# sparisi/pvr_habitat

Measured on AMD Instinct MI355X. Metric: frames/sec embedded (ResNet50, 256x256), higher is better.
Workload: dtype f16

## Files before the change

### include/pvr_hip.h

```cpp
#ifndef PVR_HIP_H
#define PVR_HIP_H

#include <stddef.h>
#include <stdint.h>

#ifdef __cplusplus
extern "C" {
#endif

typedef int pvr_status;
#define PVR_OK 0
#define PVR_ERR_INVALID 1
#define PVR_ERR_MISSING_WEIGHT 2
#define PVR_ERR_HIP 3
#define PVR_ERR_STATE 4

#define PVR_BF16 0
#define PVR_F16 1
#define PVR_F32 2

#define PVR_ARCH_RESNET50 0
#define PVR_ARCH_RESNET50_L4 1
#define PVR_ARCH_RESNET50_L3 2
#define PVR_ARCH_CLIP_VIT_B32 3
// ... 79 lines not shown
                             int32_t h, int32_t w, int32_t cin, int32_t cout, int32_t kh, int32_t kw, int32_t stride, int32_t pad, int32_t relu,
                             int32_t out_f32, int32_t dtype, void *hip_stream);
pvr_status pvr_op_conv2d_dual(const void *in_dev, const void *in2_dev, const void *wgt_dev, const float *bias_dev, void *out_dev, int32_t n, int32_t h,
                              int32_t w, int32_t cin, int32_t cout, int32_t kh, int32_t kw, int32_t stride, int32_t pad, int32_t h2, int32_t w2,
                              int32_t cin2, int32_t stride2, int32_t relu, int32_t dtype, void *hip_stream);
pvr_status pvr_op_conv_wfrag_pool(const void *in_dev, const void *wgt_packed_dev, const float *bias_dev, const void *residual_dev, float *pool_out_dev,
                                  int64_t pool_stride, int32_t n, int32_t cin, int32_t cout, int32_t dtype, void *hip_stream);
int64_t pvr_debug_conv_wfrag_launches(void);
pvr_status pvr_op_split16_pack_weights(const float *w_dev, void *out_dev, int32_t rows, int32_t k, void *hip_stream);
pvr_status pvr_op_conv2d_split16(const float *in_dev, const void *wgt_split_dev, const float *bias_dev, const float *residual_dev, float *out_dev, int32_t n,
                                 int32_t h, int32_t w, int32_t cin, int32_t cout, int32_t k, int32_t stride, int32_t pad, int32_t relu, void *hip_stream);
pvr_status pvr_op_conv2d_f32(const float *in_dev, const float *wgt_dev, const float *bias_dev, const float *residual_dev, float *out_dev, int32_t n,
                             int32_t h, int32_t w, int32_t cin, int32_t cout, int32_t k, int32_t stride, int32_t pad, int32_t relu, void *hip_stream);
int64_t pvr_debug_conv_split16_launches(void);
int64_t pvr_debug_chain_wave128_launches(void);
pvr_status pvr_debug_set_stem_regpool(int32_t mode);
pvr_status pvr_debug_set_conv_algo(int32_t algo);
pvr_status pvr_file_sizes(const char *const *paths, int32_t n, int64_t *sizes, int32_t threads);
pvr_status pvr_read_files(const char *const *paths, int32_t n, uint8_t *dst, const int64_t *offsets, int32_t threads);
pvr_status pvr_stage_copy(void *dst, const void *src, int64_t rows, int64_t row_bytes, int64_t src_row_stride, int64_t run_bytes,
                          int64_t run_stride, int32_t threads);
int64_t pvr_png_scratch_bytes(int32_t n, int32_t h, int32_t w);
pvr_status pvr_png_decode(const uint8_t *files_dev, const int64_t *offsets_dev, int32_t n, int32_t h, int32_t w, uint8_t *out_dev,
                          uint8_t *scratch_dev, int64_t scratch_bytes, int32_t *status_dev, void *hip_stream);

int64_t pvr_debug_conv_expand_launches(void);
int64_t pvr_debug_pp_persistent_launches(void);
pvr_status pvr_op_avgpool(const void *in_dev, float *out_dev, int64_t out_stride, int32_t n, int32_t hw,
                          int32_t c, int32_t in_f32, int32_t dtype, void *hip_stream);
pvr_status pvr_op_nonfinite_flag(const float *x_dev, int64_t rows, int64_t cols, int64_t stride, int32_t *flag_dev, void *hip_stream);
// ... 9 lines not shown
```

### pvr_habitat_amd/_lib.py

```python
import ctypes as C
import os

_HERE = os.path.dirname(os.path.abspath(__file__))
LIB_PATH = os.environ.get('PVR_LIB') or os.path.join(_HERE, 'lib', 'libpvr_hip.so')

PVR_BF16, PVR_F16, PVR_F32 = 0, 1, 2
ARCH_RESNET50, ARCH_RESNET50_L4, ARCH_RESNET50_L3 = 0, 1, 2


class EncoderDesc(C.Structure):
    _fields_ = [('arch', C.c_int32), ('dtype', C.c_int32), ('max_batch', C.c_int32), ('chunk', C.c_int32),
                ('resize', C.c_int32), ('crop', C.c_int32), ('mean', C.c_float * 3), ('std_', C.c_float * 3)]


_lib = None

_SIGS = {
    'pvr_version': (C.c_char_p, []),
    'pvr_has_experiments': (C.c_int32, []),
    'pvr_debug_stem_u8_geometry_ok': (C.c_int32, [C.c_void_p, C.c_int32, C.c_int32, C.c_int32, C.c_int32]),
    'pvr_encoder_set_host_backend': (C.c_int, [C.c_void_p, C.c_int32]),
    'pvr_stage_copy': (C.c_int, [C.c_void_p, C.c_void_p, C.c_int64, C.c_int64, C.c_int64, C.c_int64, C.c_int64, C.c_int32]),
    'pvr_last_error': (C.c_size_t, [C.c_char_p, C.c_size_t]),
    'pvr_encoder_create': (C.c_int, [C.POINTER(EncoderDesc), C.POINTER(C.c_void_p)]),
# ... 34 lines not shown
    'pvr_op_conv_wfrag': (C.c_int, [C.c_void_p] * 5 + [C.c_int32] * 12 + [C.c_void_p]),
    'pvr_debug_conv_wfrag_launches': (C.c_int64, []),
    'pvr_op_conv_wfrag_pool': (C.c_int, [C.c_void_p] * 5 + [C.c_int64] + [C.c_int32] * 4 + [C.c_void_p]),
    'pvr_op_conv2d_dual': (C.c_int, [C.c_void_p] * 5 + [C.c_int32] * 15 + [C.c_void_p]),
    'pvr_op_pack_frag_weights': (C.c_int, [C.c_void_p, C.c_void_p, C.c_int32, C.c_int32, C.c_void_p]),
    'pvr_debug_bneck_frame_stamps': (C.c_int, [C.c_void_p] * 12 + [C.c_int32] * 2 + [C.c_void_p] * 2),
    'pvr_encoder_check_range': (C.c_int, [C.c_void_p, C.c_void_p, C.c_int32, C.c_int32, C.c_int32, C.c_void_p, C.c_int64, C.c_void_p, C.POINTER(C.c_int32)]),
    'pvr_encoder_debug_set_switch': (C.c_int, [C.c_void_p, C.c_char_p, C.c_int32]),
    'pvr_encoder_launch_kernel': (C.c_int32, [C.c_void_p, C.c_int32, C.c_int32, C.c_char_p, C.c_int32]),
    'pvr_op_split16_pack_weights': (C.c_int, [C.c_void_p, C.c_void_p, C.c_int32, C.c_int32, C.c_void_p]),
    'pvr_op_conv2d_split16': (C.c_int, [C.c_void_p] * 5 + [C.c_int32] * 9 + [C.c_void_p]),
    'pvr_op_conv2d_f32': (C.c_int, [C.c_void_p] * 5 + [C.c_int32] * 9 + [C.c_void_p]),
    'pvr_debug_conv_split16_launches': (C.c_int64, []),
    'pvr_debug_set_stem_regpool': (C.c_int, [C.c_int32]),
    'pvr_debug_chain_wave128_launches': (C.c_int64, []),
    'pvr_op_nonfinite_flag': (C.c_int, [C.c_void_p, C.c_int64, C.c_int64, C.c_int64, C.c_void_p, C.c_void_p]),
}


def lib():
    global _lib
    if _lib is None:
        if not os.path.isfile(LIB_PATH):
            raise RuntimeError('libpvr_hip.so not found at %s: build it with `make -C pvr_habitat_amd/csrc` '
                               '(there is no CPU fallback for the HIP path)' % LIB_PATH)
        l = C.CDLL(LIB_PATH)
        for name, (res, args) in _SIGS.items():
            if not hasattr(l, name):
                continue
            f = getattr(l, name)
# ... 26 lines not shown
```

### pvr_habitat_amd/csrc/api.hip

```cpp
#include <stdarg.h>
#include "common.h"
#include "sample_rng.h"
#include <dlfcn.h>

namespace pvr {

static thread_local std::string g_err;

void set_error(const char *fmt, ...) {
    char buf[1024];
    va_list ap;
    va_start(ap, fmt);
    vsnprintf(buf, sizeof buf, fmt, ap);
    va_end(ap);
    g_err = buf;
}
const std::string &last_error() { return g_err; }

namespace {
typedef int (*roctx_push_fn)(const char *);
typedef int (*roctx_pop_fn)();
struct Roctx {
    roctx_push_fn push = nullptr;
    roctx_pop_fn pop = nullptr;
// ... 34 lines not shown
                                int dtype, hipStream_t stream, unsigned long long *stamps);
void set_frame64(int mode);
long long bneck_frame64_launches();
long long pp_persistent_launches();
pvr_status launch_conv_pp256(const void *in, const void *wgt, const float *bias, const void *res, void *out, int n, int h, int w, int cin,
                             int cout, int kh, int kw, int stride, int pad, int act, int out_f32, int res_f32, int dtype, int bm, hipStream_t stream,
                             const void *in2 = nullptr, int h2 = 0, int w2 = 0, int cin2 = 0, int stride2 = 1);
long long conv_wfrag_launches();
pvr_status launch_conv_wfrag(const void *in, const void *wp, const float *bias, const void *res, void *out, int n, int h, int w, int cin, int cout,
                             int kh, int kw, int stride, int pad, int act, int out_f32, int dtype, hipStream_t stream, float *pool_out = nullptr,
                             int64_t pool_stride = 0);

void set_stem_regpool(int v);
long long conv_split16_launches();
long long chain_wave128_launches();
pvr_status launch_split16_pack(const float *w, void *out, int rows, int K, hipStream_t stream);
pvr_status launch_conv_split16(const float *in, const void *wsp, const float *bias, const float *res, float *out, int n, int h, int w, int cin,
                               int cout, int k, int stride, int pad, int relu, hipStream_t stream, float *out2 = nullptr, int n1 = 0, void *out16 = nullptr,
                               int terms = 3);
pvr_status launch_conv_f32(const float *, const float *, const float *, const float *, float *, int, int, int, int, int, int, int, int, int, hipStream_t);

static void *g_zero = nullptr;
static pvr_status zero_page(void **out) {
    if (!g_zero) {
        PVR_HIP_TRY(hipMalloc(&g_zero, 256));
        PVR_HIP_TRY(hipMemset(g_zero, 0, 256));
        PVR_HIP_TRY(hipDeviceSynchronize());
    }
    *out = g_zero;
    return PVR_OK;
// ... 65 lines not shown
    PVR_REQUIRE(n > 0 && h > 0 && w > 0, "pvr_op_conv2d_split16: empty input");
    return launch_conv_split16(in, wgt_split, bias, residual, out, n, h, w, cin, cout, k, stride, pad, relu, (hipStream_t)stream);
}
pvr_status pvr_op_conv2d_f32(const float *in, const float *wgt, const float *bias, const float *residual, float *out, int32_t n, int32_t h, int32_t w,
                             int32_t cin, int32_t cout, int32_t k, int32_t stride, int32_t pad, int32_t relu, void *stream) {
    PVR_REQUIRE(in && wgt && bias && out && n > 0, "pvr_op_conv2d_f32: null argument");
    return launch_conv_f32(in, wgt, bias, residual, out, n, h, w, cin, cout, k, stride, pad, relu, (hipStream_t)stream);
}
int64_t pvr_debug_conv_split16_launches(void) { return (int64_t)conv_split16_launches(); }
pvr_status pvr_debug_set_stem_regpool(int32_t mode) {
    PVR_REQUIRE(mode >= -1 && mode <= 1, "pvr_debug_set_stem_regpool: -1 (environment: PVR_STEM_REGPOOL, default on), 0 (LDS-tile pooling) or 1 (register pooling)");
    set_stem_regpool(mode);
    return PVR_OK;
}
int64_t pvr_debug_chain_wave128_launches(void) { return (int64_t)chain_wave128_launches(); }
int64_t pvr_debug_pp_persistent_launches(void) { return (int64_t)pp_persistent_launches(); }

size_t pvr_last_error(char *buf, size_t cap) {
    const std::string &e = last_error();
    if (buf && cap) {
        size_t n = e.size() < cap - 1 ? e.size() : cap - 1;
        memcpy(buf, e.data(), n);
        buf[n] = 0;
    }
    return e.size();
}

pvr_status pvr_op_preprocess(const uint8_t *frames, int32_t n, int32_t h, int32_t w, int32_t resize, int32_t crop,
                             void *out, int32_t dtype, void *stream) {
    PVR_REQUIRE(frames && out, "pvr_op_preprocess: null pointer");
// ... 83 lines not shown
```

### pvr_habitat_amd/csrc/bottleneck_chain.hip

```cpp
#include "chain_params.h"

namespace pvr {


__device__ __forceinline__ void ch_dma16(__amdgpu_buffer_rsrc_t rs, char *lds, int voff, int soff) {
    __builtin_amdgcn_raw_ptr_buffer_load_lds(rs, (__attribute__((address_space(3))) void *)lds, 16, voff, soff, 0, 0);
}

#ifdef CHAIN_STAMP
__device__ unsigned long long chain_stamps[8192][12];
#define CH_T(i_) { if (threadIdx.x == 0) ch_tt[i_] = __builtin_amdgcn_s_memrealtime(); }
#else
#define CH_T(i_)
#endif

#ifndef CH_KNOCK
#define CH_KNOCK 0
#endif
template <int AUX = 0>
__device__ __forceinline__ void store_b128_imm(u32x4 v, __amdgpu_buffer_rsrc_t rs, int voff, int imm) {
    if constexpr (!(CH_KNOCK & 1)) __builtin_amdgcn_raw_buffer_store_b128(v, rs, voff + imm, 0, AUX);
}

template <int CM, int CMN, bool F16, int RD, int OCC, bool HALO, bool DS = false, int PFK = -1>
// ... 561 lines not shown
    return !e || atoi(e) != 0;
}

bool chain_uses_wave_form(int cm, int cmn, int stride, bool ds) { return chain_wave_enabled() && chain_wave_supported(cm, cmn, stride, ds); }

bool chain_uses_wave128(int cm, int cmn, int stride, int64_t M) { return chain_wave_enabled() && chain_wave128_supported(cm, cmn, stride, M); }

bool chain_ds_supported(int cm, int cmn, int cin, int stride) { return cm == 64 && cmn == 64 && cin == 64 && stride == 1; }
bool chain_supported(int cm, int cmn) { return (cm == 64 && (cmn == 0 || cmn == 64 || cmn == 128)) || (cm == 128 && (cmn == 0 || cmn == 128)); }

int chain_row_source(int row) { return (row & ~31) + 8 * ((row >> 2) & 3) + 4 * ((row >> 4) & 1) + (row & 3); }

pvr_status launch_bottleneck_chain(const void *t1, const void *w2, const float *b2, const void *w3p, const float *b3, const void *res,
                                   void *y, const void *w1np, const float *b1n, void *t1n, int n, int h, int w, int cm, int cmn,
                                   int stride, int dtype, hipStream_t stream, const void *xds, const void *wdsp, const void *w3pb, const void *wdspb,
                                   int wave, int in_blk, int out_blk, const void *wpk) {
    PVR_REQUIRE(chain_supported(cm, cmn), "bottleneck chain: unsupported widths Cm=%d next=%d", cm, cmn);
    PVR_REQUIRE(t1 && w2 && b2 && w3p && b3 && (res || xds) && y && (cmn == 0 || (w1np && b1n && t1n)), "bottleneck chain: null argument");
    PVR_REQUIRE(!xds || (wdsp && chain_ds_supported(cm, cmn, 64, stride)), "bottleneck chain with downsample: unsupported shape");
    ChainP p;
    p.in = (const u16 *)t1; p.w2 = (const u16 *)w2; p.w3 = (const u16 *)w3p; p.w1n = (const u16 *)w1np; p.res = (const u16 *)res;
    p.b2 = b2; p.b3 = b3; p.b1n = b1n; p.y = (u16 *)y; p.t1n = (u16 *)t1n;
    p.N = n; p.H = h; p.W = w; p.stride = stride;
    p.Ho = (h + 2 - 3) / stride + 1; p.Wo = (w + 2 - 3) / stride + 1;
    const int64_t M = (int64_t)n * p.Ho * p.Wo;
    const int64_t inb = (int64_t)n * h * w * cm * 2, yb = M * 4 * cm * 2, tb = M * (cmn ? cmn : 1) * 2;
    PVR_REQUIRE(inb < 0x7ffffff0ll && yb < 0x7ffffff0ll && tb < 0x7ffffff0ll, "bottleneck chain: operand larger than 2 GiB (use a smaller chunk)");
    p.M = (int)M; p.in_bytes = (unsigned)inb; p.y_bytes = (unsigned)yb; p.t1n_bytes = (unsigned)tb;
    p.xds = (const u16 *)xds; p.wds = (const u16 *)wdsp;
    p.xds_bytes = xds ? (unsigned)(M * 64 * 2) : 0; p.wds_bytes = xds ? (unsigned)(4 * cm * 64 * 2) : 0;
    p.w2_bytes = (unsigned)(cm * 9 * cm * 2); p.w3_bytes = (unsigned)(4 * cm * cm * 2); p.w1n_bytes = (unsigned)(cmn * 4 * cm * 2);
    if (wave == 2) {
        PVR_REQUIRE(chain_wave128_supported(cm, cmn, stride, M) && !xds, "bottleneck chain: no layer2 wave form for Cm=%d next=%d stride=%d", cm, cmn, stride);
        p.wpk = (const u16 *)wpk; p.in_blk = in_blk; p.out_blk = out_blk & 1;
        return launch_chain_wave128(p, cmn, dtype, stream);
    }
    if (wave) {
        PVR_REQUIRE(chain_wave_supported(cm, cmn, stride, xds != nullptr), "bottleneck chain: no wave form for Cm=%d next=%d stride=%d", cm, cmn, stride);
        p.w3b = (const u16 *)w3pb; p.wdsb = (const u16 *)wdspb; p.in_blk = in_blk; p.out_blk = out_blk;
        return launch_chain_wave(p, cmn, dtype, stream);
    }
    PVR_REQUIRE(!(in_blk || out_blk) || M % 16 == 0, "bottleneck chain: the blocked layout needs a multiple of 16 pixels");
    p.res_blk = xds ? 0 : in_blk; p.y_blk = out_blk & 1;
    p.t_blk = (out_blk & 2) && cmn > 0;
    return dtype == PVR_F16 ? launch_chain_dt<true>(p, cm, cmn, stream) : launch_chain_dt<false>(p, cm, cmn, stream);
}

}
```

### pvr_habitat_amd/csrc/chain_params.h

```cpp
#pragma once
#include "common.h"

namespace pvr {

struct ChainP {
    const u16 *in, *w2, *w3, *w1n, *res;
    const float *b2, *b3, *b1n;
    u16 *y, *t1n;
    int N, H, W, Ho, Wo, stride, M;
    unsigned in_bytes, w2_bytes, w3_bytes, w1n_bytes, y_bytes, t1n_bytes;
    const u16 *xds = nullptr, *wds = nullptr;
    unsigned xds_bytes = 0, wds_bytes = 0;
    int in_blk = 0, out_blk = 0;
    int res_blk = 0, y_blk = 0;
    const u16 *w3b = nullptr, *wdsb = nullptr;
    const u16 *wpk = nullptr;
    unsigned wpk_bytes = 0;
    int t_blk = 0;
};

bool chain_supported(int cm, int cmn);
bool chain_ds_supported(int cm, int cmn, int cin, int stride);
bool chain_uses_wave_form(int cm, int cmn, int stride, bool ds);
int chain_row_source(int row);
pvr_status launch_bottleneck_chain(const void *t1, const void *w2, const float *b2, const void *w3p, const float *b3, const void *res,
                                   void *y, const void *w1np, const float *b1n, void *t1n, int n, int h, int w, int cm, int cmn,
                                   int stride, int dtype, hipStream_t stream, const void *xds = nullptr, const void *wdsp = nullptr,
                                   const void *w3pb = nullptr, const void *wdspb = nullptr, int wave = 0, int in_blk = 0, int out_blk = 0,
                                   const void *wpk = nullptr);


bool chain_wave_supported(int cm, int cmn, int stride, bool ds);
bool chain_wave_blocked_ok(int cmn_first, int h, int w);
bool chain_wave_halo_enabled();
pvr_status launch_chain_wave(ChainP &p, int cmn, int dtype, hipStream_t stream);

bool chain_wave128_supported(int cm, int cmn, int stride, int64_t M);
bool chain_uses_wave128(int cm, int cmn, int stride, int64_t M);
size_t chain_wave128_pack_bytes();
pvr_status launch_chain_wave128_pack(const void *w2, const void *w3p, const void *w1np, void *out, hipStream_t stream);
pvr_status launch_chain_wave128(ChainP &p, int cmn, int dtype, hipStream_t stream);

}
```

### pvr_habitat_amd/csrc/chain_wave.hip

```cpp
#include "chain_params.h"

namespace pvr {

__device__ __forceinline__ int cw_row_source(int row) { return (row & ~31) + 8 * ((row >> 2) & 3) + 4 * ((row >> 4) & 1) + (row & 3); }

#ifndef CW_KNOCK
#define CW_KNOCK 0
#endif
#ifndef CW_AUX_ST
#define CW_AUX_ST PVR_NT_AUX(1)
#endif
#ifndef CW_AUX_RES
#define CW_AUX_RES PVR_NT_AUX(2)
#endif
template <int AUX = CW_AUX_ST>
__device__ __forceinline__ void cw_store(u32x4 v, __amdgpu_buffer_rsrc_t rs, int voff, int imm, int never = 0) {
    if constexpr (CW_KNOCK & 1) { if (never) __builtin_amdgcn_raw_buffer_store_b128(v, rs, voff + imm, 0, AUX); }
    else __builtin_amdgcn_raw_buffer_store_b128(v, rs, voff + imm, 0, AUX);
}
#ifndef CW_AUX_T1
#define CW_AUX_T1 CW_AUX_ST
#endif

typedef float cw_f32x2 __attribute__((ext_vector_type(2)));
// ... 20 lines not shown
__device__ __forceinline__ unsigned cw_row_shift(unsigned lo, unsigned hi, int d) {
#define CW_SH(D_) case D_: { const int a_ = __builtin_amdgcn_update_dpp(0, (int)lo, 0x100 + D_, 0xf, 0xf, true); \
                             return (unsigned)__builtin_amdgcn_update_dpp(a_, (int)hi, 0x110 + (16 - D_), 0xf, 0xf, false); }
    switch (d) {
        CW_SH(1) CW_SH(2) CW_SH(3) CW_SH(4) CW_SH(5) CW_SH(6) CW_SH(7) CW_SH(8) CW_SH(9) CW_SH(10) CW_SH(11) CW_SH(12) CW_SH(13) CW_SH(14) CW_SH(15)
        default: return lo;
    }
#undef CW_SH
}

struct CwTile {
    int xb[2];
    int mk[2];
    int yi[2];
    int yo[2];
    int to[2];
    int hb;
    int xs[2];
};

template <int CMN, bool INB, bool OUTB>
__device__ __forceinline__ void cw_setup(CwTile &a, int m0, int lane, int M, int H, int W) {
    const int fr = lane & 15, fq = lane >> 4, lp = lane >> 2, lc = (lane & 3) ^ ((lane >> 3) & 3);
    a.hb = ((m0 >> 4) - 4) * 2048 + fq * 256 + fr * 16;
#pragma unroll
    for (int j = 0; j < 2; ++j) {
        const int m = m0 + 16 * j + (INB ? fr : lp);
        const bool ok = m < M;
        const int mm = ok ? m : 0;
        const int wo = mm % W, ho = (mm / W) % H;
        int hb = 0, wb = 0;
#pragma unroll
        for (int t3 = 0; t3 < 3; ++t3) {
            hb |= (int)(ok && (unsigned)(ho - 1 + t3) < (unsigned)H) << t3;
            wb |= (int)((unsigned)(wo - 1 + t3) < (unsigned)W) << t3;
        }
        int mask = 0;
#pragma unroll
        for (int t3 = 0; t3 < 3; ++t3) mask |= ((hb >> t3) & 1) ? (wb << (t3 * 3)) : 0;
        a.mk[j] = mask;
        a.xb[j] = INB ? m : m * 128 + lc * 16;
        a.xs[j] = (m0 + 16 * j + lp) * 128 + lc * 16;
        const int blk = (m0 >> 4) + j;
        a.yi[j] = INB ? blk * 8192 + fq * 256 + fr * 16 : (m0 + 16 * j + lp) * 512 + lc * 16;
        a.yo[j] = OUTB ? blk * 8192 + fq * 256 + fr * 16 : (m0 + 16 * j + (lane >> 3)) * 512 + (((lane & 7) ^ (lane >> 3)) << 4);
        a.to[j] = OUTB ? blk * (CMN * 32) + fq * 256 + fr * 16 : (m0 + 16 * j + (lane >> 3)) * (CMN * 2) + (((lane & 7) ^ (lane >> 3)) << 4);
    }
}

template <int CMN, bool F16, bool DS, bool W3G, bool INB, bool OUTB, bool HALO, int XD, int RD, int WD>
__global__ __launch_bounds__(512, 2) void chain_wave_kernel(ChainP p) {
    typedef typename HT<F16>::V8 V8;
    constexpr int WW = 56, HB = 10;
    constexpr int NH = 8, NK = 18;
    constexpr int TN1 = CMN / 16;
    constexpr int W2L = 0, W3L = 73728, W1L = W3G ? 73728 : 73728 + 32768;
    constexpr int B2L = W1L + CMN * 512, B3L = B2L + 256, B1L = B3L + 1024, SCR = B1L + 512;
    constexpr int OOB = 0x7ffffff0;
    constexpr int YH = INB ? 1024 : 64;
    static_assert(XD >= 1 && XD <= NK && RD >= 1 && RD <= NH && NH % RD == 0 && WD >= 1 && WD <= NH, "prefetch depths (the residual ring must close over a tile)");
    static_assert(!HALO || INB, "the halo form reads the blocked layout");
    extern __shared__ __attribute__((aligned(16))) char smem[];

    const int tid = threadIdx.x, lane = tid & 63, wave = tid >> 6, fr = lane & 15, fq = lane >> 4;
    const int foff = fr * 64 + ((fq ^ ((fr >> 1) & 3)) << 4);
    char *const slot0 = smem + SCR + wave * 2048, *const slot1 = slot0 + 1024;
    const auto rs_in = __builtin_amdgcn_make_buffer_rsrc(const_cast<u16 *>(p.in), 0, p.in_bytes, 0x00020000);
    const auto rs_w2 = __builtin_amdgcn_make_buffer_rsrc(const_cast<u16 *>(p.w2), 0, p.w2_bytes, 0x00020000);
    const auto rs_w3 = __builtin_amdgcn_make_buffer_rsrc(const_cast<u16 *>(p.w3), 0, p.w3_bytes, 0x00020000);
    const auto rs_w1 = __builtin_amdgcn_make_buffer_rsrc(const_cast<u16 *>(p.w1n), 0, p.w1n_bytes, 0x00020000);
    const auto rs_res = __builtin_amdgcn_make_buffer_rsrc(const_cast<u16 *>(DS ? p.xds : p.res), 0, DS ? p.xds_bytes : p.y_bytes, 0x00020000);
    const auto rs_wd = __builtin_amdgcn_make_buffer_rsrc(const_cast<u16 *>(DS ? p.wdsb : p.w3b), 0, DS ? p.wds_bytes : p.w3_bytes, 0x00020000);
    const auto rs_y = __builtin_amdgcn_make_buffer_rsrc(p.y, 0, p.y_bytes, 0x00020000);
    const auto rs_t = __builtin_amdgcn_make_buffer_rsrc(p.t1n, 0, p.t1n_bytes, 0x00020000);

#pragma unroll
    for (int q = 0; q < 9; ++q) {
        const int r = tid >> 3, c = tid & 7;
        const u32x4 v = __builtin_bit_cast(u32x4, __builtin_amdgcn_raw_buffer_load_b128(rs_w2, (cw_row_source(r) * 576 + c * 8) * 2, q * 128, 0));
        *reinterpret_cast<u32x4 *>(smem + W2L + q * 8192 + r * 128 + ((c ^ ((r >> 1) & 7)) << 4)) = v;
    }
    if constexpr (!W3G) {
#pragma unroll
        for (int q = 0; q < 4; ++q) {
            const int idx = tid + 512 * q, r = idx >> 3, c = idx & 7;
            const u32x4 v = __builtin_bit_cast(u32x4, __builtin_amdgcn_raw_buffer_load_b128(rs_w3, idx * 16, 0, 0));
            *reinterpret_cast<u32x4 *>(smem + W3L + r * 128 + ((c ^ ((r >> 1) & 7)) << 4)) = v;
        }
// ... 8 lines not shown
    }
    if (tid < 64) *reinterpret_cast<float *>(smem + B2L + tid * 4) = p.b2[tid];
    if (tid < 256) *reinterpret_cast<float *>(smem + B3L + tid * 4) = p.b3[tid];
    if constexpr (CMN > 0) { if (tid < CMN) *reinterpret_cast<float *>(smem + B1L + tid * 4) = p.b1n[tid]; }
    __syncthreads();

    const int nch = (p.M + 255) >> 8, cx = (nch + 7) >> 3, L = gridDim.x >> 3;
    const int xcd = blockIdx.x & 7, c_end = min((xcd + 1) * cx, nch);
    int chunk = xcd * cx + (blockIdx.x >> 3);
    if (chunk >= c_end) return;

    int lb0 = fr * 128 + ((fq ^ ((fr >> 1) & 7)) << 4), lb1 = lb0 ^ 64;
    const int Wb = p.W * 128;

    CwTile cur, nxt;
    cw_setup<CMN, INB, OUTB>(cur, chunk * 256 + wave * 32, lane, p.M, p.H, p.W);

    u32x4 xr[HALO ? 1 : XD][2];
    u32x4 xh[HALO ? HB : 1][2];
    u32x4 rres[DS ? 1 : RD][2];
    V8 xd[2][2];
    u32x4 wg[(W3G || DS) ? WD : 1][2][2];
#define CW_ISSUE_X(slot_, kt_, A_)                                                                                      \
    {                                                                                                                   \
        const int tp_ = (kt_) >> 1;                                                                                     \
        _Pragma("unroll") for (int j = 0; j < 2; ++j) {                                                                 \
            int vo_;                                                                                                    \
            if constexpr (INB) {                                   \
                const int pm_ = A_.xb[j] + (tp_ / 3 - 1) * p.W + (tp_ % 3 - 1);                                         \
                vo_ = (pm_ >> 4) * 2048 + (pm_ & 15) * 16 + (((kt_) & 1) * 4 + fq) * 256;                               \
            } else vo_ = A_.xb[j] + (tp_ / 3 - 1) * Wb + (tp_ % 3 - 1) * 128 + ((kt_) & 1) * 64;                        \
// ... 93 lines not shown
        for (int q = 0; q < 2; ++q) {
            const float4 bA = *reinterpret_cast<const float4 *>(smem + B2L + (32 * q + 8 * fq) * 4);
            const float4 bB = *reinterpret_cast<const float4 *>(smem + B2L + (32 * q + 8 * fq + 4) * 4);
#pragma unroll
            for (int j = 0; j < 2; ++j) {
                const f32x4 lo = acc2[2 * q][j], hi = acc2[2 * q + 1][j];
                const float v[8] = {lo[0] + bA.x, lo[1] + bA.y, lo[2] + bA.z, lo[3] + bA.w, hi[0] + bB.x, hi[1] + bB.y, hi[2] + bB.z, hi[3] + bB.w};
                u32x4 o;
#pragma unroll
                for (int e = 0; e < 4; ++e)
                    o[e] = cw_pack2<F16>(fmaxf(v[2 * e], 0.f), fmaxf(v[2 * e + 1], 0.f));
                t2[q][j] = o;
            }
        }

        cw_setup<CMN, INB, OUTB>(nxt, more ? chunk_n * 256 + wave * 32 : ((p.M + 31) & ~31), lane, p.M, p.H, p.W);
        if (!more) nxt.hb = OOB;
        if constexpr (HALO) CW_ISSUE_HALO(nxt)
        else {
#pragma unroll
            for (int k = 0; k < XD; ++k) CW_ISSUE_X(k, k, nxt);
        }
        if constexpr (W3G || DS) {
#pragma unroll
            for (int d = 0; d < WD; ++d) CW_ISSUE_WG(d, d);
        }
        if constexpr (DS) {
#pragma unroll
            for (int ks = 0; ks < 2; ++ks)
#pragma unroll
                for (int j = 0; j < 2; ++j) xd[ks][j] = __builtin_bit_cast(V8, cw_m2f(j ? slot1 : slot0, lane, foff, xdr[ks][j]));
// ... 65 lines not shown
#pragma unroll
                    for (int e = 0; e < 4; ++e) {
                        const float v0 = fmaxf(v[2 * e] + from_h<F16>((u16)(r[e] & 0xffffu)), 0.f);
                        const float v1 = fmaxf(v[2 * e + 1] + from_h<F16>((u16)(r[e] >> 16)), 0.f);
                        o[j][e] = cw_pack2<F16>(v0, v1);
                    }
                }
            }
#pragma unroll
            for (int j = 0; j < 2; ++j) {
                if constexpr (OUTB) cw_store(o[j], rs_y, cur.yo[j], h * 1024, p.stride == 77);
                else if (h & 1) {
                    u32x4 lo, hi;
                    cw_f2m_pair(slot0, lane, oe[j], o[j], lo, hi);
                    cw_store(lo, rs_y, cur.yo[j], (h >> 1) * 128, p.stride == 77);
                    cw_store(hi, rs_y, cur.yo[j], (h >> 1) * 128 + 8 * 512, p.stride == 77);
                } else oe[j] = o[j];
            }
            if constexpr (CMN > 0) {
#pragma unroll
                for (int i = 0; i < TN1; ++i) {
                    const V8 wb = *reinterpret_cast<const V8 *>(smem + W1L + (h >> 1) * (CMN * 128) + i * 2048 + ((h & 1) ? lb1 : lb0));
#pragma unroll
                    for (int j = 0; j < 2; ++j) acc1[i][j] = mfma16<F16>(wb, __builtin_bit_cast(V8, o[j]), acc1[i][j]);
                }
            }
            __builtin_amdgcn_sched_barrier(0);
        }

        if constexpr (CMN > 0) {
            u32x4 te[2];
// ... 86 lines not shown
        return launch_cw_one<0, F16, false, false, false, false, false, 4, 4, 1>(p, stream);
    }
    set_error("bottleneck chain (wave form): no instance for next Cm=%d%s, blocked in/out %d/%d", cmn, p.xds ? " with downsample" : "", (int)ib, (int)ob);
    return PVR_ERR_INVALID;
}

bool chain_wave_supported(int cm, int cmn, int stride, bool ds) {
    if (cm != 64 || stride != 1) return false;
    if (ds) return cmn == 64;
    if (cmn == 128) { const char *e = getenv("PVR_CHAIN_WAVE_128"); return !e || atoi(e) != 0; }
    return cmn == 0 || cmn == 64;
}

bool chain_wave_blocked_ok(int cmn_first, int h, int w) { return cmn_first == 64 && (h * w) % 32 == 0; }
bool chain_wave_halo_enabled() { return cw_halo() != 0; }

pvr_status launch_chain_wave(ChainP &p, int cmn, int dtype, hipStream_t stream) {
    PVR_REQUIRE((int64_t)(p.M + 64) * 512 < 0x7ffffff0ll, "bottleneck chain (wave form): operand larger than 2 GiB (use a smaller chunk)");
    PVR_REQUIRE(p.xds ? p.wdsb != nullptr : (cmn != 128 || p.w3b != nullptr), "bottleneck chain (wave form): the blocked copy of W3 / Wd is missing");
    PVR_REQUIRE(!(p.in_blk || p.out_blk) || p.M % 32 == 0, "bottleneck chain (wave form): the blocked layout needs a multiple of 32 pixels");
    return dtype == PVR_F16 ? launch_cw_dt<true>(p, cmn, stream) : launch_cw_dt<false>(p, cmn, stream);
}

}
```

### pvr_habitat_amd/csrc/encoder.hip

```cpp
#include "encoder_internal.h"

namespace pvr {

pvr_status launch_split16_pack(const float *w, void *out, int rows, int K, hipStream_t stream);
bool conv_split16_supported(int cin, int cout, int k);
pvr_status launch_conv_split16(const float *in, const void *wsp, const float *bias, const float *res, float *out, int n, int h, int w, int cin,
                               int cout, int k, int stride, int pad, int relu, hipStream_t stream, float *out2 = nullptr, int n1 = 0, void *out16 = nullptr,
                               int terms = 3);

static void read_switches(PlanSwitches &sw) {
    auto get = [](const char *name, int def) { const char *v = getenv(name); return v ? atoi(v) : def; };
    sw.pool_fuse = get("PVR_POOL_FUSE", 1);
    sw.stem_u8 = get("PVR_STEM_U8", 1);
    sw.stem_lds = get("PVR_STEM_LDS", 1);
    sw.frame_front1 = get("PVR_FRAME_FRONT1", 1);
    sw.frame_next1 = get("PVR_FRAME_NEXT1", 0);
    sw.dual_ds = get("PVR_DUAL_DS", 1);
    sw.chain_ds = get("PVR_CHAIN_DS", 1);
    sw.chain_blocked = get("PVR_CHAIN_BLOCKED", 1);
    sw.splitk = get("PVR_SPLITK", 1);
    sw.smallk_div = get("PVR_SMALLK_DIV", 4);
    if (sw.smallk_div < 1) sw.smallk_div = 1;
    sw.frame_min_n = get("PVR_FRAME_MIN_N", 128);
    sw.frame_run = get("PVR_FRAME_RUN", 0);
    sw.frame_stagger = get("PVR_FRAME_RUN_STAGGER", 0);
    sw.split16 = get("PVR_SPLIT16", 1);
    sw.stem_conv1 = get("PVR_STEM_CONV1", 1);
    sw.resid32 = get("PVR_RESID32", 1);
    sw.tail_f32 = get("PVR_TAIL_F32", 1);
    sw.fuse = get("PVR_FUSE", 1);
}

template <bool F32>
__global__ __launch_bounds__(256) void range_flag_kernel(const void *x, size_t n8, int dtype, int *flags, int idx) {
    bool bad = false;
    for (size_t i = (size_t)blockIdx.x * 256 + threadIdx.x; i < n8; i += (size_t)gridDim.x * 256) {
        if constexpr (F32) {
            const u32x4 a = reinterpret_cast<const u32x4 *>(x)[2 * i], b = reinterpret_cast<const u32x4 *>(x)[2 * i + 1];
#pragma unroll
            for (int e = 0; e < 4; ++e) bad |= (a[e] & 0x7f800000u) == 0x7f800000u || (b[e] & 0x7f800000u) == 0x7f800000u;
        } else {
            const u32x4 a = reinterpret_cast<const u32x4 *>(x)[i];
            const unsigned em = dtype == PVR_F16 ? 0x7c00u : 0x7f80u;
#pragma unroll
            for (int e = 0; e < 4; ++e) bad |= ((a[e] & em) == em) || (((a[e] >> 16) & em) == em);
// ... 557 lines not shown
    if (e->sw.stem_conv1 && !e->sched_fused.empty() && (e->desc.arch == PVR_ARCH_RESNET50 || e->desc.arch == PVR_ARCH_RESNET50_L3 || e->desc.arch == PVR_ARCH_RESNET50_L4)) {
        const Launch &L0 = e->sched_fused[0];
        if (L0.conv3 < 0 && L0.ds < 0 && L0.pair < 0 && !L0.frame && L0.conv2 == 0) {
            const ConvOp &c1 = e->ops[0];
            if (c1.kind == 0 && !c1.f32op && !c1.from32 && c1.k == 1 && c1.stride == 1 && c1.cin == 64 && c1.cout == 64 && c1.cin_real == 64 && c1.cout_real == 64 && c1.relu == 1 &&
                c1.in_buf == B_X0 && c1.out_buf == B_T1 && c1.res_buf == B_NONE && !c1.out_f32 && c1.tap.empty() && c1.ksplit <= 1 && c1.h == 56 && (int)c1.h_w.size() == 64 * 64) {
                std::vector<u16> img(64 * 64);
                stem_c1_pack(c1.h_w.data(), img.data());
                pvr_status s = enc_upload(&e->d_stem_c1w, img);
                if (s) return s;
                e->stem_c1 = 0; e->stem_c1_blk = L0.out_blk;
                e->sched_fused.erase(e->sched_fused.begin());
            }
        }
    }
    return PVR_OK;
}

static pvr_status finalize_stem(pvr_encoder *e, const std::string &conv_name = "conv1.weight", const std::string &bn_name = "bn1",
                                int cout_real = 64, int ks = 7) {
    const HostTensor *w;
    pvr_status s;
    if ((s = enc_need(e, conv_name, &w, (size_t)cout_real * 3 * ks * ks))) return s;
    std::vector<float> scale, shift;
    if ((s = bn_fold(e, bn_name, cout_real, scale, shift))) return s;
    scale.resize(64, 0.f); shift.resize(64, 0.f);
    const int t0 = (7 - ks) / 2;
    auto wat = [&](int co, int c, int a, int b) -> double {
        const int aa = a - t0, bb = b - t0;
        if (co >= cout_real || aa < 0 || aa >= ks || bb < 0 || bb >= ks) return 0.0;
// ... 402 lines not shown
                s = launch_conv_expand(enc->d_buf[c1.in_buf], c1.d_w, c1.d_b, nullptr, enc->d_buf[c1.out_buf], nb, c1.h, c1.w, c1.cin, c1.cout, 1, c1.relu, dt, st, 1);
                t1_blocked = true;
            } else
                s = launch_conv(enc->d_buf[c1.in_buf], c1.d_w, c1.d_b, nullptr, enc->d_buf[c1.out_buf], enc->d_zero, nb, c1.h, c1.w, c1.cin, c1.cout, 1, 1, 1, 0, c1.relu, 0, dt, st);
            if (s) return s;
        }
        bool pooled = false;
        const std::vector<Launch> &plan_ = cur_plan(enc);
        if (enc->kinds_algo != conv_algo() || enc->kinds_stride != plan_.size()) resolve_kinds(enc);
        const uint8_t *kinds = enc->kinds.data() + (size_t)(nb - 1) * plan_.size();
        float *smallk = enc->d_smallk[enc->cur_lane];
        const bool pool_args_ok = enc->stop_after.empty() && out_stride % 4 == 0 && (((size_t)(out + (size_t)f0 * out_stride)) & 15) == 0;
        int launch_idx = 0;
        const bool run_ok = enc->stop_after.empty() && !enc->range_flags;
        const int stop_idx = enc->stop_after.size() > 1 && enc->stop_after[0] == '#' ? atoi(enc->stop_after.c_str() + 1) : -1;
        auto member = [&](const ConvOp &o, const void *in, const void *r_, void *out_) -> pvr_status {
            if (const int ks = small_batch_ksplit(enc, o, nb)) {
                if (!smallk) { set_error("low-latency plan without its scratch (pvr_encoder_set_low_latency allocates it)"); return PVR_ERR_STATE; }
                return launch_conv_splitk(in, o.d_w, o.d_b, r_, out_, enc->d_zero, smallk, ks, nb, o.h, o.w, o.cin, o.cout, o.k, o.k, o.stride, o.pad, o.relu, o.out_f32, dt, st);
            }
            return launch_conv(in, o.d_w, o.d_b, r_, out_, enc->d_zero, nb, o.h, o.w, o.cin, o.cout, o.k, o.k, o.stride, o.pad, o.relu, o.out_f32, dt, st);
        };
        for (size_t li = 0; li < plan_.size(); ++li) {
            const Launch &l = plan_[li];
            const ConvOp &op = enc->ops[l.conv3 >= 0 ? l.conv3 : l.conv2];
            const void *res = op.res_buf == B_NONE ? nullptr : enc->d_buf[op.res_buf];
            int kind = kinds[li];
            if (kind == LK_WFRAG_POOL && !pool_args_ok) kind = resolve_kind(enc, plan_, li, nb, false);
            if ((kind == LK_FRAME_RUN || kind == LK_FRAME_RUN_TAIL) && !run_ok) kind = LK_FRAME_FRONT1;
            switch (kind) {
            case LK_FRAME_RUN: {
                BFBlk blks[6];
                int nblk = 0;
                for (size_t t = li; t < plan_.size() && nblk < 6 && (t == li || kinds[t] == LK_FRAME_RUN_TAIL); ++t, ++nblk) {
                    const Launch &lt = plan_[t];
                    const ConvOp &o3 = enc->ops[lt.conv3], &o2 = enc->ops[lt.conv2], &o1 = enc->ops[lt.conv1];
                    blks[nblk] = BFBlk{(const u16 *)o1.d_wfb, (const u16 *)o2.d_wfb, (const u16 *)o3.d_wfb, (const u16 *)enc->d_buf[o3.res_buf], o1.d_b, o2.d_b, o3.d_b,
                                       (u16 *)enc->d_buf[o3.out_buf]};
                }
                s = launch_bneck_frame_run(blks, nblk, nb, dt, st, enc->sw.frame_stagger);
                break;
            }
            case LK_FRAME_RUN_TAIL:
// ... 32 lines not shown
            }
            case LK_DUAL_MEMBERS: {
                const ConvOp &cd = enc->ops[l.ds];
                s = member(cd, enc->d_buf[cd.in_buf], nullptr, enc->d_buf[cd.out_buf]);
                if (!s) s = member(op, enc->d_buf[op.in_buf], res, enc->d_buf[op.out_buf]);
                break;
            }
            case LK_CHAIN: {
                const ConvOp &c2 = enc->ops[l.conv2];
                const ConvOp *c1 = l.next1 >= 0 ? &enc->ops[l.next1] : nullptr;
                const ConvOp *cd = l.ds >= 0 ? &enc->ops[l.ds] : nullptr;
                s = launch_bottleneck_chain(enc->d_buf[l.t1_in], c2.d_w, c2.d_b, op.d_wp, cd ? op.d_bsum : op.d_b, res, enc->d_buf[op.out_buf],
                                            c1 ? c1->d_wp : nullptr, c1 ? c1->d_b : nullptr, c1 ? enc->d_buf[l.t1_out] : nullptr, nb,
                                            c2.h, c2.w, c2.cout, c1 ? c1->cout : 0, c2.stride, dt, st,
                                            cd ? enc->d_buf[cd->in_buf] : nullptr, cd ? cd->d_wp : nullptr, op.d_wpb, cd ? cd->d_wpb : nullptr,
                                            l.wave, cd ? (l.in_blk && t1_blocked) : l.in_blk, l.out_blk, c2.d_wpk);
                t1_blocked = false;
                break;
            }
            case LK_CAST:
                s = launch_f32_to_h((const float *)enc->d_buf[op.in_buf], enc->d_buf[op.out_buf], (size_t)nb * op.h * op.w * op.cin, dt, st);
                break;
            case LK_F32:
                s = launch_conv_f32((const float *)enc->d_buf[op.in_buf], op.d_wf, op.d_b, (const float *)res, (float *)enc->d_buf[op.out_buf], nb,
                                    op.h, op.w, op.cin, op.cout, op.k, op.stride, op.pad, op.relu, st);
                break;
            case LK_SPLIT16:
                s = launch_conv_split16((const float *)enc->d_buf[op.in_buf], op.d_wsp, op.d_b, (const float *)res, (float *)enc->d_buf[op.out_buf], nb,
                                        op.h, op.w, op.cin, op.cout, op.k, op.stride, op.pad, op.relu, st);
                break;
            case LK_SPLIT16_PAIR: {
// ... 15 lines not shown
                break;
            case LK_EXPAND_BLOCKED:
                s = launch_conv_expand(enc->d_buf[op.in_buf], op.d_w, op.d_b, nullptr, enc->d_buf[op.out_buf], nb, op.h, op.w, op.cin, op.cout, 1, op.relu, dt, st, 1);
                t1_blocked = true;
                break;
            case LK_WFRAG_POOL:
                s = launch_conv_wfrag(enc->d_buf[op.in_buf], op.d_wfb, op.d_b, res, nullptr, nb, op.h, op.w, op.cin, op.cout, 1, 1, 1, 0, 1, 1, dt, st,
                                      out + (size_t)f0 * out_stride, out_stride);
                pooled = true;
                break;
            case LK_WFRAG:
                s = launch_conv_wfrag(enc->d_buf[op.in_buf], op.d_wfb, op.d_b, res, enc->d_buf[op.out_buf], nb, op.h, op.w, op.cin, op.cout, op.k, op.k,
                                      op.stride, op.pad, op.relu, op.out_f32, dt, st);
                break;
            default:
                s = launch_conv(enc->d_buf[op.in_buf], op.d_w, op.d_b, res, enc->d_buf[op.out_buf], enc->d_zero, nb, op.h, op.w,
                                op.cin, op.cout, op.k, op.k, op.stride, op.pad, op.relu, op.out_f32, dt, st);
            }
            if (s) return s;
            if (enc->range_flags && kind != LK_WFRAG_POOL) {
                const int ho_ = (op.h + 2 * op.pad - op.k) / op.stride + 1, wo_ = (op.w + 2 * op.pad - op.k) / op.stride + 1;
                const size_t n8 = (size_t)nb * ho_ * wo_ * op.cout / 8;
                const int blocks = (int)((n8 + 255) / 256 < 2048 ? (n8 + 255) / 256 : 2048);
                if ((op.out_f32 & 1) || op.f32op) hipLaunchKernelGGL(range_flag_kernel<true>, dim3(blocks), dim3(256), 0, st, enc->d_buf[op.out_buf], n8, dt, enc->range_flags, (int)li);
                else hipLaunchKernelGGL(range_flag_kernel<false>, dim3(blocks), dim3(256), 0, st, enc->d_buf[op.out_buf], n8, dt, enc->range_flags, (int)li);
            }
            if ((s = mark())) return s;
            if (!enc->stop_after.empty() && op.tap == enc->stop_after) { stopped = true; break; }
            if (launch_idx++ == stop_idx) { stopped = true; break; }
        }
        enc->last_pooled = pooled;
        if (stopped) return PVR_OK;
// ... 313 lines not shown
```

### pvr_habitat_amd/csrc/encoder_internal.h

```cpp
#pragma once
#include <map>
#include <string>
#include <vector>
#include <cmath>
#include "common.h"
#include "chain_params.h"

namespace pvr {

pvr_status launch_preprocess(const uint8_t *, int, int, int, int, int, void *, int, hipStream_t, int crop_pos = 0);
pvr_status launch_stem(const void *, const void *, const float *, void *, int, int, int, hipStream_t);
pvr_status launch_maxpool(const void *, void *, int, int, int, int, int, hipStream_t);
pvr_status launch_stem_pool(const void *, const void *, const float *, void *, int, int, int, hipStream_t, const void *c1_w = nullptr, const float *c1_b = nullptr,
                            void *c1_t1 = nullptr, int c1_blk = 0);
bool stem_pool_u8_ok(const void *, int, int, int, int);
pvr_status launch_stem_pool_u8(const uint8_t *, int, int, int, int, int, const void *, const float *, void *, int, hipStream_t, const void *c1_w = nullptr,
                               const float *c1_b = nullptr, void *c1_t1 = nullptr, int c1_blk = 0);
bool stem_conv1_capable();
void stem_c1_pack(const u16 *w, u16 *img);
void preprocess_geometry(int h, int w, int resize, int crop, int crop_pos, int *resize_needed, int *top, int *left);
pvr_status launch_avgpool(const void *, float *, int64_t, int, int, int, int, int, hipStream_t);
pvr_status launch_nhwc_to_chw(const float *, float *, int64_t, int, int, int, int, hipStream_t);
pvr_status launch_h_to_f32(const void *, float *, size_t, int, hipStream_t);
pvr_status launch_f32_to_h(const float *, void *, size_t, int, hipStream_t);
// ... 66 lines not shown
    float *d_bsum = nullptr;
    u16 *d_wcat = nullptr;
    std::string tap;
    int ksplit = 0, ks_buf = B_NONE;
};

struct Launch {
    int conv2 = -1, conv3 = -1, next1 = -1;
    int ds = -1;
    int t1_in = B_NONE, t1_out = B_NONE;
    int wave = 0;
    int conv1 = -1;
    int frame = 0;
    int pair = -1;
    int in_blk = 0, out_blk = 0;
};

enum LaunchKind : uint8_t {
    LK_CONV = 0,
    LK_FRAME_FRONT1,
    LK_FRAME,
    LK_FRAME_RUN,
    LK_FRAME_RUN_TAIL,
    LK_FRAME_MEMBERS,
    LK_DUAL,
    LK_DUAL_MEMBERS,
    LK_CHAIN,
    LK_CAST,
    LK_F32,
    LK_SPLIT16,
// ... 14 lines not shown
    int frame_front1 = 1;
    int frame_next1 = 0;
    int dual_ds = 1;
    int chain_ds = 1;
    int chain_blocked = 1;
    int splitk = 1;
    int smallk_div = 4;
    int frame_run = 0;
    int frame_stagger = 0;
    int frame_min_n = 128;
    int stem_conv1 = 1;
    int split16 = 1;
    int resid32 = 1;
    int tail_f32 = 1;
    int fuse = 1;
};

}

using namespace pvr;

namespace pvr { struct HostPlan; }

struct pvr_encoder {
    pvr_encoder_desc desc;
    std::map<std::string, HostTensor> weights;
    std::vector<ConvOp> ops;
    std::vector<Launch> sched_plain, sched_fused;
    bool fuse = true;
    bool low_latency = false;
// ... 73 lines not shown
```

Measured before the change: 97820.

## Store only stride-2 subsampled chain output when its sole reader is a strided 1x1 conv

When a wave-form bottleneck chain's output y is read only by 1x1 stride-2 convs before being overwritten, the chain now writes just the even-row, even-column pixels into a compact tensor. The downstream conv then runs as a stride-1 conv on the half-resolution input. This cuts y write bandwidth by about 4x and lets the reader do contiguous loads. It adds a planner pass that scans for readers and writers, plus extra address arithmetic per store in the chain kernel.

```diff
diff --git a/include/pvr_hip.h b/include/pvr_hip.h
--- a/include/pvr_hip.h
+++ b/include/pvr_hip.h
@@ -117,6 +117,7 @@
                              int32_t h, int32_t w, int32_t cin, int32_t cout, int32_t k, int32_t stride, int32_t pad, int32_t relu, void *hip_stream);
 int64_t pvr_debug_conv_split16_launches(void);
 int64_t pvr_debug_chain_wave128_launches(void);
+int64_t pvr_debug_strided_y_launches(void);
 pvr_status pvr_debug_set_stem_regpool(int32_t mode);
 pvr_status pvr_debug_set_conv_algo(int32_t algo);
 pvr_status pvr_file_sizes(const char *const *paths, int32_t n, int64_t *sizes, int32_t threads);
diff --git a/pvr_habitat_amd/_lib.py b/pvr_habitat_amd/_lib.py
--- a/pvr_habitat_amd/_lib.py
+++ b/pvr_habitat_amd/_lib.py
@@ -72,6 +72,7 @@
     'pvr_debug_conv_split16_launches': (C.c_int64, []),
     'pvr_debug_set_stem_regpool': (C.c_int, [C.c_int32]),
     'pvr_debug_chain_wave128_launches': (C.c_int64, []),
+    'pvr_debug_strided_y_launches': (C.c_int64, []),
     'pvr_op_nonfinite_flag': (C.c_int, [C.c_void_p, C.c_int64, C.c_int64, C.c_int64, C.c_void_p, C.c_void_p]),
 }
 
diff --git a/pvr_habitat_amd/csrc/api.hip b/pvr_habitat_amd/csrc/api.hip
--- a/pvr_habitat_amd/csrc/api.hip
+++ b/pvr_habitat_amd/csrc/api.hip
@@ -72,6 +72,7 @@
 void set_stem_regpool(int v);
 long long conv_split16_launches();
 long long chain_wave128_launches();
+long long strided_y_launches();
 pvr_status launch_split16_pack(const float *w, void *out, int rows, int K, hipStream_t stream);
 pvr_status launch_conv_split16(const float *in, const void *wsp, const float *bias, const float *res, float *out, int n, int h, int w, int cin,
                                int cout, int k, int stride, int pad, int relu, hipStream_t stream, float *out2 = nullptr, int n1 = 0, void *out16 = nullptr,
@@ -167,6 +168,7 @@
     return PVR_OK;
 }
 int64_t pvr_debug_chain_wave128_launches(void) { return (int64_t)chain_wave128_launches(); }
+int64_t pvr_debug_strided_y_launches(void) { return (int64_t)strided_y_launches(); }
 int64_t pvr_debug_pp_persistent_launches(void) { return (int64_t)pp_persistent_launches(); }
 
 size_t pvr_last_error(char *buf, size_t cap) {
diff --git a/pvr_habitat_amd/csrc/bottleneck_chain.hip b/pvr_habitat_amd/csrc/bottleneck_chain.hip
--- a/pvr_habitat_amd/csrc/bottleneck_chain.hip
+++ b/pvr_habitat_amd/csrc/bottleneck_chain.hip
@@ -599,7 +599,7 @@
 pvr_status launch_bottleneck_chain(const void *t1, const void *w2, const float *b2, const void *w3p, const float *b3, const void *res,
                                    void *y, const void *w1np, const float *b1n, void *t1n, int n, int h, int w, int cm, int cmn,
                                    int stride, int dtype, hipStream_t stream, const void *xds, const void *wdsp, const void *w3pb, const void *wdspb,
-                                   int wave, int in_blk, int out_blk, const void *wpk) {
+                                   int wave, int in_blk, int out_blk, const void *wpk, int y_s2) {
     PVR_REQUIRE(chain_supported(cm, cmn), "bottleneck chain: unsupported widths Cm=%d next=%d", cm, cmn);
     PVR_REQUIRE(t1 && w2 && b2 && w3p && b3 && (res || xds) && y && (cmn == 0 || (w1np && b1n && t1n)), "bottleneck chain: null argument");
     PVR_REQUIRE(!xds || (wdsp && chain_ds_supported(cm, cmn, 64, stride)), "bottleneck chain with downsample: unsupported shape");
@@ -623,8 +623,10 @@
     if (wave) {
         PVR_REQUIRE(chain_wave_supported(cm, cmn, stride, xds != nullptr), "bottleneck chain: no wave form for Cm=%d next=%d stride=%d", cm, cmn, stride);
         p.w3b = (const u16 *)w3pb; p.wdsb = (const u16 *)wdspb; p.in_blk = in_blk; p.out_blk = out_blk;
+        p.y_s2 = y_s2; p.ys2_bytes = y_s2 ? (unsigned)((int64_t)n * (h / 2) * (w / 2) * 4 * cm * 2) : 0;
         return launch_chain_wave(p, cmn, dtype, stream);
     }
+    PVR_REQUIRE(!y_s2, "bottleneck chain: strided y is built for the wave form only");
     PVR_REQUIRE(!(in_blk || out_blk) || M % 16 == 0, "bottleneck chain: the blocked layout needs a multiple of 16 pixels");
     p.res_blk = xds ? 0 : in_blk; p.y_blk = out_blk & 1;
     p.t_blk = (out_blk & 2) && cmn > 0;
diff --git a/pvr_habitat_amd/csrc/chain_params.h b/pvr_habitat_amd/csrc/chain_params.h
--- a/pvr_habitat_amd/csrc/chain_params.h
+++ b/pvr_habitat_amd/csrc/chain_params.h
@@ -17,6 +17,8 @@
     const u16 *wpk = nullptr;
     unsigned wpk_bytes = 0;
     int t_blk = 0;
+    int y_s2 = 0;
+    unsigned ys2_bytes = 0;
 };
 
 bool chain_supported(int cm, int cmn);
@@ -27,7 +29,8 @@
                                    void *y, const void *w1np, const float *b1n, void *t1n, int n, int h, int w, int cm, int cmn,
                                    int stride, int dtype, hipStream_t stream, const void *xds = nullptr, const void *wdsp = nullptr,
                                    const void *w3pb = nullptr, const void *wdspb = nullptr, int wave = 0, int in_blk = 0, int out_blk = 0,
-                                   const void *wpk = nullptr);
+                                   const void *wpk = nullptr, int y_s2 = 0);
+bool chain_wave_strided_y_ok(int cmn, int h, int w);
 
 
 bool chain_wave_supported(int cm, int cmn, int stride, bool ds);
diff --git a/pvr_habitat_amd/csrc/chain_wave.hip b/pvr_habitat_amd/csrc/chain_wave.hip
--- a/pvr_habitat_amd/csrc/chain_wave.hip
+++ b/pvr_habitat_amd/csrc/chain_wave.hip
@@ -58,13 +58,16 @@
     int mk[2];
     int yi[2];
     int yo[2];
+    int yh[2];
     int to[2];
     int hb;
     int xs[2];
 };
 
+constexpr int CW_Y_SKIP = 0x7fff0000;
+
 template <int CMN, bool INB, bool OUTB>
-__device__ __forceinline__ void cw_setup(CwTile &a, int m0, int lane, int M, int H, int W) {
+__device__ __forceinline__ void cw_setup(CwTile &a, int m0, int lane, int M, int H, int W, int ys2 = 0) {
     const int fr = lane & 15, fq = lane >> 4, lp = lane >> 2, lc = (lane & 3) ^ ((lane >> 3) & 3);
     a.hb = ((m0 >> 4) - 4) * 2048 + fq * 256 + fr * 16;
 #pragma unroll
@@ -88,6 +91,18 @@
         const int blk = (m0 >> 4) + j;
         a.yi[j] = INB ? blk * 8192 + fq * 256 + fr * 16 : (m0 + 16 * j + lp) * 512 + lc * 16;
         a.yo[j] = OUTB ? blk * 8192 + fq * 256 + fr * 16 : (m0 + 16 * j + (lane >> 3)) * 512 + (((lane & 7) ^ (lane >> 3)) << 4);
+        if constexpr (CMN == 128 && !OUTB) {
+            a.yh[j] = a.yo[j] + 8 * 512;
+            if (ys2) {
+#pragma unroll
+                for (int r = 0; r < 2; ++r) {
+                    const int ms = m0 + 16 * j + 8 * r + (lane >> 3), ws = ms % W, ts = ms / W, hs = ts % H, ns = ts / H;
+                    const int o = (ms < M && !((hs | ws) & 1)) ? ((ns * (H >> 1) + (hs >> 1)) * (W >> 1) + (ws >> 1)) * 512 + (((lane & 7) ^ (lane >> 3)) << 4) : CW_Y_SKIP;
+                    if (r) a.yh[j] = o;
+                    else a.yo[j] = o;
+                }
+            }
+        }
         a.to[j] = OUTB ? blk * (CMN * 32) + fq * 256 + fr * 16 : (m0 + 16 * j + (lane >> 3)) * (CMN * 2) + (((lane & 7) ^ (lane >> 3)) << 4);
     }
 }
@@ -115,7 +130,7 @@
     const auto rs_w1 = __builtin_amdgcn_make_buffer_rsrc(const_cast<u16 *>(p.w1n), 0, p.w1n_bytes, 0x00020000);
     const auto rs_res = __builtin_amdgcn_make_buffer_rsrc(const_cast<u16 *>(DS ? p.xds : p.res), 0, DS ? p.xds_bytes : p.y_bytes, 0x00020000);
     const auto rs_wd = __builtin_amdgcn_make_buffer_rsrc(const_cast<u16 *>(DS ? p.wdsb : p.w3b), 0, DS ? p.wds_bytes : p.w3_bytes, 0x00020000);
-    const auto rs_y = __builtin_amdgcn_make_buffer_rsrc(p.y, 0, p.y_bytes, 0x00020000);
+    const auto rs_y = __builtin_amdgcn_make_buffer_rsrc(p.y, 0, (CMN == 128 && !OUTB && p.y_s2) ? p.ys2_bytes : p.y_bytes, 0x00020000);
     const auto rs_t = __builtin_amdgcn_make_buffer_rsrc(p.t1n, 0, p.t1n_bytes, 0x00020000);
 
 #pragma unroll
@@ -154,7 +169,7 @@
     const int Wb = p.W * 128;
 
     CwTile cur, nxt;
-    cw_setup<CMN, INB, OUTB>(cur, chunk * 256 + wave * 32, lane, p.M, p.H, p.W);
+    cw_setup<CMN, INB, OUTB>(cur, chunk * 256 + wave * 32, lane, p.M, p.H, p.W, p.y_s2);
 
     u32x4 xr[HALO ? 1 : XD][2];
     u32x4 xh[HALO ? HB : 1][2];
@@ -278,7 +293,7 @@
             }
         }
 
-        cw_setup<CMN, INB, OUTB>(nxt, more ? chunk_n * 256 + wave * 32 : ((p.M + 31) & ~31), lane, p.M, p.H, p.W);
+        cw_setup<CMN, INB, OUTB>(nxt, more ? chunk_n * 256 + wave * 32 : ((p.M + 31) & ~31), lane, p.M, p.H, p.W, p.y_s2);
         if (!more) nxt.hb = OOB;
         if constexpr (HALO) CW_ISSUE_HALO(nxt)
         else {
@@ -374,7 +389,8 @@
                     u32x4 lo, hi;
                     cw_f2m_pair(slot0, lane, oe[j], o[j], lo, hi);
                     cw_store(lo, rs_y, cur.yo[j], (h >> 1) * 128, p.stride == 77);
-                    cw_store(hi, rs_y, cur.yo[j], (h >> 1) * 128 + 8 * 512, p.stride == 77);
+                    if constexpr (CMN == 128) cw_store(hi, rs_y, cur.yh[j], (h >> 1) * 128, p.stride == 77);
+                    else cw_store(hi, rs_y, cur.yo[j], (h >> 1) * 128 + 8 * 512, p.stride == 77);
                 } else oe[j] = o[j];
             }
             if constexpr (CMN > 0) {
@@ -491,11 +507,17 @@
 
 bool chain_wave_blocked_ok(int cmn_first, int h, int w) { return cmn_first == 64 && (h * w) % 32 == 0; }
 bool chain_wave_halo_enabled() { return cw_halo() != 0; }
+bool chain_wave_strided_y_ok(int cmn, int h, int w) { return cmn == 128 && h % 2 == 0 && w % 2 == 0; }
+
+static long long g_strided_y_launches = 0;
+long long strided_y_launches() { return g_strided_y_launches; }
 
 pvr_status launch_chain_wave(ChainP &p, int cmn, int dtype, hipStream_t stream) {
     PVR_REQUIRE((int64_t)(p.M + 64) * 512 < 0x7ffffff0ll, "bottleneck chain (wave form): operand larger than 2 GiB (use a smaller chunk)");
     PVR_REQUIRE(p.xds ? p.wdsb != nullptr : (cmn != 128 || p.w3b != nullptr), "bottleneck chain (wave form): the blocked copy of W3 / Wd is missing");
     PVR_REQUIRE(!(p.in_blk || p.out_blk) || p.M % 32 == 0, "bottleneck chain (wave form): the blocked layout needs a multiple of 32 pixels");
+    PVR_REQUIRE(!p.y_s2 || (chain_wave_strided_y_ok(cmn, p.H, p.W) && !p.out_blk && !p.xds && p.stride == 1), "bottleneck chain (wave form): strided y needs Cmn = 128, NHWC out, even H and W");
+    if (p.y_s2) ++g_strided_y_launches;
     return dtype == PVR_F16 ? launch_cw_dt<true>(p, cmn, stream) : launch_cw_dt<false>(p, cmn, stream);
 }
 
diff --git a/pvr_habitat_amd/csrc/encoder.hip b/pvr_habitat_amd/csrc/encoder.hip
--- a/pvr_habitat_amd/csrc/encoder.hip
+++ b/pvr_habitat_amd/csrc/encoder.hip
@@ -29,6 +29,7 @@
     sw.resid32 = get("PVR_RESID32", 1);
     sw.tail_f32 = get("PVR_TAIL_F32", 1);
     sw.fuse = get("PVR_FUSE", 1);
+    sw.strided_y = get("PVR_STRIDED_Y", 1);
 }
 
 template <bool F32>
@@ -616,6 +617,40 @@
             }
         }
     }
+    if (e->sw.strided_y) {
+        std::vector<Launch> &sc = e->sched_fused;
+        for (size_t a = 0; a < sc.size(); ++a) {
+            Launch &P = sc[a];
+            if (P.conv3 < 0 || P.frame || P.wave != 1 || P.next1 < 0 || P.ds >= 0 || P.out_blk) continue;
+            const ConvOp &p2 = e->ops[P.conv2], &p3 = e->ops[P.conv3];
+            if (p2.stride != 1 || !chain_wave_strided_y_ok(e->ops[P.next1].cout, p3.h, p3.w)) continue;
+            const int yb = p3.out_buf;
+            auto reads = [&](int oi) { return oi >= 0 && (e->ops[oi].in_buf == yb || e->ops[oi].res_buf == yb); };
+            auto writes = [&](int oi) { return oi >= 0 && e->ops[oi].out_buf == yb; };
+            auto s2_reader = [&](int oi) {
+                const ConvOp &o = e->ops[oi];
+                return o.kind == 0 && !o.f32op && !o.from32 && !o.d_wfb && o.k == 1 && o.stride == 2 && o.pad == 0 && o.in_buf == yb && o.res_buf != yb &&
+                       o.h == p3.h && o.w == p3.w && o.cin == p3.cout && o.cin_real == o.cin && o.ksplit <= 1 &&
+                       o.k * o.k * o.cin < 512;
+            };
+            std::vector<size_t> rd;
+            bool ok = true, closed = false;
+            for (size_t b = a + 1; b < sc.size() && ok && !closed; ++b) {
+                const Launch &L = sc[b];
+                const int members[5] = {L.conv1, L.conv2, L.conv3, L.ds, L.pair};
+                bool r = L.t1_in == yb, w = L.t1_out == yb || writes(L.next1);
+                for (int oi : members) { r = r || reads(oi); w = w || writes(oi); }
+                if (r) {
+                    if (L.conv3 < 0 && L.ds < 0 && L.pair < 0 && L.conv1 < 0 && !L.frame && !L.out_blk && s2_reader(L.conv2)) rd.push_back(b);
+                    else ok = false;
+                }
+                closed = w;
+            }
+            if (!ok || !closed || rd.empty()) continue;
+            P.y_s2 = 1;
+            for (size_t b : rd) sc[b].in_s2 = 1;
+        }
+    }
     return PVR_OK;
 }
 
@@ -1048,6 +1083,7 @@
         int launch_idx = 0;
         const bool run_ok = enc->stop_after.empty() && !enc->range_flags;
         const int stop_idx = enc->stop_after.size() > 1 && enc->stop_after[0] == '#' ? atoi(enc->stop_after.c_str() + 1) : -1;
+        const bool s2_on = enc->stop_after.empty();
         auto member = [&](const ConvOp &o, const void *in, const void *r_, void *out_) -> pvr_status {
             if (const int ks = small_batch_ksplit(enc, o, nb)) {
                 if (!smallk) { set_error("low-latency plan without its scratch (pvr_encoder_set_low_latency allocates it)"); return PVR_ERR_STATE; }
@@ -1060,7 +1096,9 @@
             const ConvOp &op = enc->ops[l.conv3 >= 0 ? l.conv3 : l.conv2];
             const void *res = op.res_buf == B_NONE ? nullptr : enc->d_buf[op.res_buf];
             int kind = kinds[li];
+            const bool in_s2 = l.in_s2 && s2_on;
             if (kind == LK_WFRAG_POOL && !pool_args_ok) kind = resolve_kind(enc, plan_, li, nb, false);
+            if (in_s2 && kind != LK_CONV) { set_error("strided y: launch %zu reads the compact tensor but runs as %s", li, launch_kind_name(kind)); return PVR_ERR_STATE; }
             if ((kind == LK_FRAME_RUN || kind == LK_FRAME_RUN_TAIL) && !run_ok) kind = LK_FRAME_FRONT1;
             switch (kind) {
             case LK_FRAME_RUN: {
@@ -1123,7 +1161,7 @@
                                             c1 ? c1->d_wp : nullptr, c1 ? c1->d_b : nullptr, c1 ? enc->d_buf[l.t1_out] : nullptr, nb,
                                             c2.h, c2.w, c2.cout, c1 ? c1->cout : 0, c2.stride, dt, st,
                                             cd ? enc->d_buf[cd->in_buf] : nullptr, cd ? cd->d_wp : nullptr, op.d_wpb, cd ? cd->d_wpb : nullptr,
-                                            l.wave, cd ? (l.in_blk && t1_blocked) : l.in_blk, l.out_blk, c2.d_wpk);
+                                            l.wave, cd ? (l.in_blk && t1_blocked) : l.in_blk, l.out_blk, c2.d_wpk, l.y_s2 && s2_on);
                 t1_blocked = false;
                 break;
             }
@@ -1169,8 +1207,8 @@
                                       op.stride, op.pad, op.relu, op.out_f32, dt, st);
                 break;
             default:
-                s = launch_conv(enc->d_buf[op.in_buf], op.d_w, op.d_b, res, enc->d_buf[op.out_buf], enc->d_zero, nb, op.h, op.w,
-                                op.cin, op.cout, op.k, op.k, op.stride, op.pad, op.relu, op.out_f32, dt, st);
+                s = launch_conv(enc->d_buf[op.in_buf], op.d_w, op.d_b, res, enc->d_buf[op.out_buf], enc->d_zero, nb, in_s2 ? op.h / 2 : op.h, in_s2 ? op.w / 2 : op.w,
+                                op.cin, op.cout, op.k, op.k, in_s2 ? 1 : op.stride, op.pad, op.relu, op.out_f32, dt, st);
             }
             if (s) return s;
             if (enc->range_flags && kind != LK_WFRAG_POOL) {
diff --git a/pvr_habitat_amd/csrc/encoder_internal.h b/pvr_habitat_amd/csrc/encoder_internal.h
--- a/pvr_habitat_amd/csrc/encoder_internal.h
+++ b/pvr_habitat_amd/csrc/encoder_internal.h
@@ -104,6 +104,8 @@
     int frame = 0;
     int pair = -1;
     int in_blk = 0, out_blk = 0;
+    int y_s2 = 0;
+    int in_s2 = 0;
 };
 
 enum LaunchKind : uint8_t {
@@ -148,6 +150,7 @@
     int resid32 = 1;
     int tail_f32 = 1;
     int fuse = 1;
+    int strided_y = 1;
 };
 
 }
```

After: 99200 (median of 6 runs). +1.4%, better.
